# aiforvision/OCTA-autosegmentation

Measured on AMD Instinct MI355X. Metric: synthetic OCTA samples/sec (graph + 304x304 image + 1216x1216 label triples), higher is better.
Workload: dtype f64

## Files before the change

include/octa_hip.h:

```cpp
#ifndef OCTA_HIP_H
#define OCTA_HIP_H

#include <stddef.h>
#include <stdint.h>

#ifdef __cplusplus
extern "C" {
#endif

typedef struct octa_ctx octa_ctx;


int octa_abi_version(void);

const char *octa_last_error(void);

int octa_ctx_create(int device, octa_ctx **out);
void octa_ctx_destroy(octa_ctx *ctx);

size_t octa_ctx_scratch_bytes(const octa_ctx *ctx);

int octa_rasterize_2d(octa_ctx *ctx, int B, const double *d_edges, const int64_t *h_edge_off,
                      const uint8_t *d_keep, int no_pixels_x, int no_pixels_y, int mip_axis,
                      double min_radius, double max_radius, uint8_t *d_out, void *stream);
// ... 252 lines not shown

int octa_sim_edge_offsets(octa_sim *sim, int64_t *h_edge_off, int64_t *h_n_art);

int octa_sim_export_edges(octa_sim *sim, double *h_edges);

int octa_sim_export_edges_device(octa_sim *sim, double *d_edges, void *stream);

int octa_sim_trace(octa_sim *sim, int32_t *h_trace);

int octa_sim_stats(octa_sim *sim, int64_t *h_stats);

int octa_sim_kd_paths(octa_sim *sim, int64_t *h_paths);

int octa_sim_assign_paths(octa_sim *sim, int64_t *h_paths);

int octa_sim_spans(octa_sim *sim, int64_t *h_spans);

int octa_sim_timing(octa_sim *sim, double *h_out8);

int octa_sim_service_stats(octa_sim *sim, double *h_out5);

int octa_sim_geometry(int num_cus, int *h_out4);

int octa_sim_is_large(const octa_sim *sim);

int octa_sim_fields(octa_sim *sim, int sample, double *h_oxy, int64_t cap_oxy, int64_t *n_oxy, double *h_co2,
                    int64_t cap_co2, int64_t *n_co2);

int octa_sim_kat_kd_order(octa_ctx *ctx, const double *h_pts, int64_t n, const uint8_t *h_need, int32_t *h_indices);

// ... 5 lines not shown
```

octa_autosegmentation_amd/_native.py:

```python
import contextlib
import ctypes
import os
import random as _random
import threading

import numpy as np

HERE = os.path.dirname(os.path.abspath(__file__))
LIB_PATH = os.environ.get("OCTA_HIP_LIB") or os.path.join(HERE, "liboctahip.so")

_lib = None
_ctxs = {}
_lock = threading.Lock()

c_void_p, c_int, c_double, c_size_t = ctypes.c_void_p, ctypes.c_int, ctypes.c_double, ctypes.c_size_t


def _struct(name, ints, ptrs):
    fields = [("struct_size", ctypes.c_uint32)] + [(k, c_int) for k in ints.split()] + [("slope", ctypes.c_float)] + [(k, c_void_p) for k in ptrs.split()]
    return type(name, (ctypes.Structure,), {"_fields_": fields})


Conv3x3Args = _struct("Conv3x3Args", "N H W Cin Cout stride in_dilation tap_mask out_scale out_off_y out_off_x C1 CY1 nslot",
                      "d_x d_x2 d_w d_y d_y2 d_scale1 d_shift1 d_scale2 d_shift2 d_stat_partials d_stat_slots d_residual")
# ... 50 lines not shown
    "octa_sim_run_states": (c_int, [c_void_p, c_void_p, c_void_p, c_void_p, c_void_p, c_void_p, c_void_p, c_void_p]),
    "octa_sim_np_state": (c_int, [c_void_p, c_int, c_void_p]),
    "octa_thinconv_expand": (c_int, [c_void_p, c_void_p, c_void_p, c_void_p, c_void_p, c_int, c_int, c_int, c_int, c_int, c_int, c_int, ctypes.c_float, c_void_p]),
    "octa_thinconv_squeeze": (c_int, [c_void_p, c_void_p, c_void_p, c_void_p, c_void_p, c_int, c_int, c_int, c_int, c_int, c_int, c_int, c_void_p]),
    "octa_lrelu_bwd_bf16": (c_int, [c_void_p, c_void_p, c_void_p, c_void_p, ctypes.c_int64, ctypes.c_float, c_void_p]),
    "octa_thinconv_wgrad_scratch_floats": (ctypes.c_longlong, [c_int, c_int, c_int, c_int]),
    "octa_thinconv_wgrad": (c_int, [c_void_p, c_void_p, c_void_p, c_void_p, c_void_p, c_void_p, c_int, c_int, c_int, c_int, c_int, c_int, c_int, c_int, c_int, c_void_p]),
    "octa_sim_spans": (c_int, [c_void_p, c_void_p]),
    "octa_sim_edge_offsets": (c_int, [c_void_p, c_void_p, c_void_p]),
    "octa_sim_export_edges": (c_int, [c_void_p, c_void_p]),
    "octa_sim_export_edges_device": (c_int, [c_void_p, c_void_p, c_void_p]),
    "octa_sim_trace": (c_int, [c_void_p, c_void_p]),
    "octa_sim_stats": (c_int, [c_void_p, c_void_p]),
    "octa_sim_kd_paths": (c_int, [c_void_p, c_void_p]),
    "octa_sim_assign_paths": (c_int, [c_void_p, c_void_p]),
    "octa_sim_timing": (c_int, [c_void_p, c_void_p]),
    "octa_sim_service_stats": (c_int, [c_void_p, c_void_p]),
    "octa_sim_geometry": (c_int, [c_int, c_void_p]),
    "octa_sim_is_large": (c_int, [c_void_p]),
    "octa_conv2d_f32_nchw": (c_int, [c_void_p, c_void_p, c_void_p, c_void_p, c_void_p] + [c_int] * 14 + [c_void_p]),
    "octa_convtranspose2x2_f32_nchw": (c_int, [c_void_p, c_void_p, c_void_p, c_void_p, c_int, c_int, c_int, c_int, c_int, c_void_p]),
    "octa_conv2d_f32_dgrad_nchw": (c_int, [c_void_p, c_void_p, c_void_p, c_void_p] + [c_int] * 11 + [c_void_p]),
    "octa_conv2d_f32_wgrad_workspace": (c_int, [c_int] * 10 + [ctypes.POINTER(c_size_t)]),
    "octa_conv2d_f32_wgrad_nchw": (c_int, [c_void_p, c_void_p, c_void_p, c_void_p, c_void_p, c_void_p, c_size_t] + [c_int] * 10 + [c_void_p]),
    "octa_sim_fields": (c_int, [c_void_p, c_int, c_void_p, ctypes.c_int64, c_void_p, c_void_p, ctypes.c_int64, c_void_p]),
    "octa_instnorm_lrelu_nhwc_bwd": (c_int, [c_void_p, c_void_p, c_void_p, c_void_p, c_void_p, c_void_p, c_void_p, c_void_p, c_void_p, c_void_p, c_int, c_int, ctypes.c_int64, ctypes.c_float, c_void_p]),
    "octa_pack_conv_weights": (c_int, [c_void_p, c_void_p, c_int, c_void_p, c_void_p]),
    "octa_head1_nhwc_bwd": (c_int, [c_void_p, c_void_p, c_void_p, c_void_p, ctypes.c_int64, c_int, c_void_p, c_void_p, c_void_p, c_void_p]),
    "octa_instnorm_nhwc_stats": (c_int, [c_void_p, c_void_p, c_void_p, c_void_p, c_void_p, c_void_p, c_void_p, c_void_p, c_int, c_int, ctypes.c_int64, ctypes.c_float, c_void_p]),
    "octa_scale_shift_lrelu_nhwc": (c_int, [c_void_p, c_void_p, c_void_p, c_void_p, c_void_p, c_int, c_int, ctypes.c_int64, ctypes.c_float, c_void_p]),
# ... 168 lines not shown
```

octa_autosegmentation_amd/csrc/sim.hip:

```cpp

#include <chrono>
#include <vector>

#include "common.h"
#include "sim_host.h"
#include <thread>
#include <atomic>
#include <cstdlib>
#include <cstring>

using namespace OCTA_SIMK;

#if OCTA_SIM_LARGE
#define OCTA_SIM_T octa_simL_impl
#define OCTA_SIM_FN(name) octa_simL_##name
#else
#define OCTA_SIM_T octa_simS_impl
#define OCTA_SIM_FN(name) octa_simS_##name
#endif
#define octa_sim_create OCTA_SIM_FN(create)
#define octa_sim_destroy OCTA_SIM_FN(destroy)
#define octa_sim_run OCTA_SIM_FN(run)
#define octa_sim_run_states OCTA_SIM_FN(run_states)
#define octa_sim_np_state OCTA_SIM_FN(np_state)
#define octa_sim_edge_offsets OCTA_SIM_FN(edge_offsets)
#define octa_sim_export_edges OCTA_SIM_FN(export_edges)
#define octa_sim_export_edges_device OCTA_SIM_FN(export_edges_device)
#define octa_sim_trace OCTA_SIM_FN(trace)
#define octa_sim_stats OCTA_SIM_FN(stats)
#define octa_sim_kd_paths OCTA_SIM_FN(kd_paths)
#define octa_sim_assign_paths OCTA_SIM_FN(assign_paths)
#define octa_sim_fields OCTA_SIM_FN(fields)
#define octa_sim_service_stats OCTA_SIM_FN(service_stats)
#define octa_sim_geometry OCTA_SIM_FN(geometry)
#define octa_sim_spans OCTA_SIM_FN(spans)
#define octa_sim_timing OCTA_SIM_FN(timing)
#define octa_sim_kat_kd_order OCTA_SIM_FN(kat_kd_order)
struct OCTA_SIM_T;
extern "C" void octa_sim_destroy(OCTA_SIM_T *S);
extern "C" long long octa_sim_next_ticket(void);
extern "C" int *octa_sim_launch_flag(int device);

namespace {

constexpr int SIM_THREADS = SIM_THREADS_PER_WG;
constexpr int SIM_WG_PER_CU = 2;
// ... 7 lines not shown
static_assert(SIM_THREADS == 64 * KD_WAVES, "kd mailboxes are sized for KD_WAVES waves");
constexpr int REQ_CAP = 8192;

static_assert(sizeof(BifRequest) == sizeof(octa_bif_request), "request layout must match the public header");
static_assert(MAXKEPT == OCTA_BIF_MAX_ATTS, "request capacity must match the public header");

struct BatchPtrs {
    double *npos[2], *nrad[2], *nkap[2];
    int *npar[2], *nch0[2], *nch1[2];
    unsigned char *nnch[2], *nact[2];
    double *oxy, *co2, *cand, *py_u;
    unsigned *py_state;
    int *nn, *act_list;
    int *nn_prev[2];
    double *nn_d2[2];
    unsigned *sorted;
    int *gnode, *gstart, *gcount;
    Rec *rec;
    int *glist, *child_group;
    FlushRec *fl_rec;
    idx_t *kd_idx, *kd_rank;
    unsigned char *removed, *ven_near;
    unsigned long long *hashes;
    unsigned *pairs;
    unsigned long long *set_hash;
    int *set_key, *tmp_int;
    double *grid_pts;
    unsigned *cand_idx;
    double *tmp_dbl;
    SampleScalars *sc;
// ... 17 lines not shown
};

__device__ __forceinline__ SimArrays sample_arrays(const BatchPtrs &B, int s) {
    SimArrays A;
    for (int f = 0; f < 2; f++) {
        A.npos[f] = B.npos[f] + (size_t)s * NCAP * 3;
        A.nrad[f] = B.nrad[f] + (size_t)s * NCAP;
        A.nkap[f] = B.nkap[f] + (size_t)s * NCAP;
        A.npar[f] = B.npar[f] + (size_t)s * NCAP;
        A.nch0[f] = B.nch0[f] + (size_t)s * NCAP;
        A.nch1[f] = B.nch1[f] + (size_t)s * NCAP;
        A.nnch[f] = B.nnch[f] + (size_t)s * NCAP;
        A.nact[f] = B.nact[f] + (size_t)s * NCAP;
        A.nn_prev[f] = B.nn_prev[f] + (size_t)s * OCAP;
        A.nn_d2[f] = B.nn_d2[f] + (size_t)s * OCAP;
    }
    A.oxy = B.oxy + (size_t)s * OCAP * 3;
    A.co2 = B.co2 + (size_t)s * CCAP * 3;
    A.cand = B.cand + (size_t)s * NCANDCAP * 3;
    A.py_u = B.py_u + (size_t)s * PYCAP;
    A.nn = B.nn + (size_t)s * OCAP;
    A.act_list = B.act_list + (size_t)s * NCAP;
    A.sorted = B.sorted + (size_t)s * SORTCAP;
    A.gnode = B.gnode + (size_t)s * GCAP;
    A.gstart = B.gstart + (size_t)s * GCAP;
    A.gcount = B.gcount + (size_t)s * GCAP;
    A.rec = B.rec + (size_t)s * GCAP;
    A.glist = B.glist + (size_t)s * GCAP;
    A.child_group = B.child_group + (size_t)s * NCAP;
    A.fl_rec = B.fl_rec + (size_t)s * 2 * MURRAY_FLUSH_LDS;
// ... 589 lines not shown
    }
    if ((nw == 0 && cfg.forest_type == 0) || cfg.n_trees < 1 || 2 * cfg.n_trees > NCAP) { octa::set_error("octa_sim_create: bad forest config"); delete S; return -2; }
    if (std::ceil(cfg.sx * 76) > 76 || std::ceil(cfg.sy * 76) > 76) { octa::set_error("octa_sim_create: simulation space larger than the unit square"); delete S; return -2; }
    S->iters = build_iter_table(cfg, &S->C);
    BatchPtrs &P = S->P;
    memset(&P, 0, sizeof(P));
    P.C = S->C;
    const size_t nb = (size_t)B;
    int rc = 0;
    for (int f = 0; f < 2 && !rc; f++) {
        rc |= dev_alloc(S, &P.npos[f], nb * NCAP * 3); rc |= dev_alloc(S, &P.nrad[f], nb * NCAP); rc |= dev_alloc(S, &P.nkap[f], nb * NCAP);
        rc |= dev_alloc(S, &P.npar[f], nb * NCAP); rc |= dev_alloc(S, &P.nch0[f], nb * NCAP); rc |= dev_alloc(S, &P.nch1[f], nb * NCAP);
        rc |= dev_alloc(S, &P.nnch[f], nb * NCAP); rc |= dev_alloc(S, &P.nact[f], nb * NCAP);
        rc |= dev_alloc(S, &P.nn_prev[f], nb * OCAP); rc |= dev_alloc(S, &P.nn_d2[f], nb * OCAP);
    }
    rc |= dev_alloc(S, &P.oxy, nb * OCAP * 3); rc |= dev_alloc(S, &P.co2, nb * CCAP * 3);
    rc |= dev_alloc(S, &P.cand, nb * NCANDCAP * 3); rc |= dev_alloc(S, &P.py_u, nb * PYCAP); rc |= dev_alloc(S, &P.py_state, nb * 625);
    rc |= dev_alloc(S, &P.nn, nb * OCAP); rc |= dev_alloc(S, &P.act_list, nb * NCAP);
    rc |= dev_alloc(S, &P.sorted, nb * SORTCAP); rc |= dev_alloc(S, &P.gnode, nb * GCAP); rc |= dev_alloc(S, &P.gstart, nb * GCAP);
    rc |= dev_alloc(S, &P.gcount, nb * GCAP); rc |= dev_alloc(S, &P.rec, nb * GCAP);
    rc |= dev_alloc(S, &P.glist, nb * GCAP); rc |= dev_alloc(S, &P.child_group, nb * NCAP); rc |= dev_alloc(S, &P.fl_rec, nb * 2 * MURRAY_FLUSH_LDS);
    rc |= dev_alloc(S, &P.kd_idx, nb * OCAP); rc |= dev_alloc(S, &P.kd_rank, nb * OCAP);
    rc |= dev_alloc(S, &P.removed, nb * OCAP); rc |= dev_alloc(S, &P.ven_near, nb * OCAP); rc |= dev_alloc(S, &P.hashes, nb * OCAP);
    rc |= dev_alloc(S, &P.pairs, nb * PCAP); rc |= dev_alloc(S, &P.set_hash, nb * SETCAP); rc |= dev_alloc(S, &P.set_key, nb * SETCAP);
    rc |= dev_alloc(S, &P.grid_pts, nb * GRID_N * 3); rc |= dev_alloc(S, &P.cand_idx, nb * NCANDCAP);
    rc |= dev_alloc(S, &P.tmp_int, nb * (OCAP + 2 * NCANDCAP)); rc |= dev_alloc(S, &P.tmp_dbl, nb * OCAP * 3);
    rc |= dev_alloc(S, &P.sc, nb); rc |= dev_alloc(S, &P.iters, S->iters.size() + 1);
    rc |= dev_alloc(S, &P.reqs, (size_t)2 * REQ_CAP); rc |= dev_alloc(S, &P.req_count, 4); rc |= dev_alloc(S, &P.bif_results, (size_t)2 * REQ_CAP * 6);
    rc |= dev_alloc(S, &P.mt_state, nb * 625); rc |= dev_alloc(S, &P.valid_count, nb);
    if (cfg.fixed()) {
// ... 525 lines not shown
        o[0] = sc.err; o[1] = sc.py_pos; o[2] = sc.murray_steps; o[3] = sc.n_bif; o[4] = sc.respec;
        o[5] = sc.n_nodes[0]; o[6] = sc.n_nodes[1];
        memcpy(&o[7], &sc.faz_radius, 8);
        for (int k = 0; k < 16; k++) o[8 + k] = sc.prof[k];
        for (int k = 0; k < 8; k++) o[24 + k] = sc.kdprof[k];
    }
    return 0;
}

extern "C" int octa_sim_kd_paths(OCTA_SIM_T *S, int64_t *h_paths) {
    if (!S || !S->ran || !h_paths) { octa::set_error("octa_sim_kd_paths: run the simulation first"); return -2; }
    for (int s = 0; s < S->B; s++) { h_paths[2 * s] = S->h_sc[s].kd_path[0]; h_paths[2 * s + 1] = S->h_sc[s].kd_path[1]; }
    return 0;
}

extern "C" int octa_sim_assign_paths(OCTA_SIM_T *S, int64_t *h_paths) {
    if (!S || !S->ran || !h_paths) { octa::set_error("octa_sim_assign_paths: run the simulation first"); return -2; }
    for (int s = 0; s < S->B; s++) { h_paths[2 * s] = S->h_sc[s].assign_path[0]; h_paths[2 * s + 1] = S->h_sc[s].assign_path[1]; }
    return 0;
}

extern "C" int octa_sim_fields(OCTA_SIM_T *S, int sample, double *h_oxy, int64_t cap_oxy, int64_t *n_oxy, double *h_co2,
                               int64_t cap_co2, int64_t *n_co2) {
    if (!S || !S->ran || sample < 0 || sample >= S->B) { octa::set_error("octa_sim_fields: bad arguments"); return -2; }
    OCTA_HIP_CHECK(hipSetDevice(S->ctx->device));
    const SampleScalars &sc = S->h_sc[sample];
    if (n_oxy) *n_oxy = sc.n_oxy;
    if (n_co2) *n_co2 = sc.n_co2;
    if (h_oxy) {
        int64_t n = sc.n_oxy < cap_oxy ? sc.n_oxy : cap_oxy;
// ... 75 lines not shown
```

octa_autosegmentation_amd/csrc/sim_api.cpp:

```cpp
#include <cstdlib>
#include <cstring>
#include <new>

#include "common.h"

extern "C" {
struct octa_simS_impl;
struct octa_simL_impl;
#define OCTA_DECL(SFX, T)                                                                                                                       \
    int octa_sim##SFX##_create(octa_ctx *, const octa_sim_config *, int, T **);                                                                 \
    void octa_sim##SFX##_destroy(T *);                                                                                                          \
    int octa_sim##SFX##_run(T *, const uint32_t *, const uint64_t *, octa_bif_fn, void *, void *);                                              \
    int octa_sim##SFX##_run_states(T *, const double *, const double *, const uint32_t *, const uint32_t *, octa_bif_fn, void *, void *);       \
    int octa_sim##SFX##_np_state(T *, int, uint32_t *);                                                                                         \
    int octa_sim##SFX##_edge_offsets(T *, int64_t *, int64_t *);                                                                                \
    int octa_sim##SFX##_export_edges(T *, double *);                                                                                            \
    int octa_sim##SFX##_export_edges_device(T *, double *, void *);                                                                             \
    int octa_sim##SFX##_trace(T *, int32_t *);                                                                                                  \
    int octa_sim##SFX##_stats(T *, int64_t *);                                                                                                  \
    int octa_sim##SFX##_kd_paths(T *, int64_t *);                                                                                               \
    int octa_sim##SFX##_assign_paths(T *, int64_t *);                                                                                           \
    int octa_sim##SFX##_spans(T *, int64_t *);                                                                                                  \
    int octa_sim##SFX##_timing(T *, double *);                                                                                                  \
    int octa_sim##SFX##_service_stats(T *, double *);                                                                                           \
    int octa_sim##SFX##_geometry(int, int *);                                                                                                   \
    int octa_sim##SFX##_fields(T *, int, double *, int64_t, int64_t *, double *, int64_t, int64_t *);
OCTA_DECL(S, octa_simS_impl)
OCTA_DECL(L, octa_simL_impl)
#undef OCTA_DECL
int octa_simS_kat_kd_order(octa_ctx *, const double *, int64_t, const uint8_t *, int32_t *);
}

#include <atomic>
#include <mutex>
static std::atomic<long long> g_sim_launches{0};
extern "C" long long octa_sim_next_ticket(void) { return g_sim_launches.fetch_add(1, std::memory_order_acq_rel) + 1; }
// ... 57 lines not shown
extern "C" int octa_sim_run(octa_sim *sim, const uint32_t *a, const uint64_t *b, octa_bif_fn f, void *u, void *st) {
    NEED(sim, "octa_sim_run") return FWD(octa_simS_run(sim->s, a, b, f, u, st), octa_simL_run(sim->l, a, b, f, u, st));
}
extern "C" int octa_sim_run_states(octa_sim *sim, const double *fz, const double *stp, const uint32_t *a, const uint32_t *b, octa_bif_fn f, void *u, void *st) {
    NEED(sim, "octa_sim_run_states") return FWD(octa_simS_run_states(sim->s, fz, stp, a, b, f, u, st), octa_simL_run_states(sim->l, fz, stp, a, b, f, u, st));
}
extern "C" int octa_sim_np_state(octa_sim *sim, int k, uint32_t *o) { NEED(sim, "octa_sim_np_state") return FWD(octa_simS_np_state(sim->s, k, o), octa_simL_np_state(sim->l, k, o)); }
extern "C" int octa_sim_edge_offsets(octa_sim *sim, int64_t *a, int64_t *b) { NEED(sim, "octa_sim_edge_offsets") return FWD(octa_simS_edge_offsets(sim->s, a, b), octa_simL_edge_offsets(sim->l, a, b)); }
extern "C" int octa_sim_export_edges(octa_sim *sim, double *e) { NEED(sim, "octa_sim_export_edges") return FWD(octa_simS_export_edges(sim->s, e), octa_simL_export_edges(sim->l, e)); }
extern "C" int octa_sim_export_edges_device(octa_sim *sim, double *e, void *st) {
    NEED(sim, "octa_sim_export_edges_device") return FWD(octa_simS_export_edges_device(sim->s, e, st), octa_simL_export_edges_device(sim->l, e, st));
}
extern "C" int octa_sim_trace(octa_sim *sim, int32_t *t) { NEED(sim, "octa_sim_trace") return FWD(octa_simS_trace(sim->s, t), octa_simL_trace(sim->l, t)); }
extern "C" int octa_sim_stats(octa_sim *sim, int64_t *t) { NEED(sim, "octa_sim_stats") return FWD(octa_simS_stats(sim->s, t), octa_simL_stats(sim->l, t)); }
extern "C" int octa_sim_kd_paths(octa_sim *sim, int64_t *t) { NEED(sim, "octa_sim_kd_paths") return FWD(octa_simS_kd_paths(sim->s, t), octa_simL_kd_paths(sim->l, t)); }
extern "C" int octa_sim_assign_paths(octa_sim *sim, int64_t *t) { NEED(sim, "octa_sim_assign_paths") return FWD(octa_simS_assign_paths(sim->s, t), octa_simL_assign_paths(sim->l, t)); }
extern "C" int octa_sim_spans(octa_sim *sim, int64_t *t) { NEED(sim, "octa_sim_spans") return FWD(octa_simS_spans(sim->s, t), octa_simL_spans(sim->l, t)); }
extern "C" int octa_sim_timing(octa_sim *sim, double *t) { NEED(sim, "octa_sim_timing") return FWD(octa_simS_timing(sim->s, t), octa_simL_timing(sim->l, t)); }
extern "C" int octa_sim_service_stats(octa_sim *sim, double *t) { NEED(sim, "octa_sim_service_stats") return FWD(octa_simS_service_stats(sim->s, t), octa_simL_service_stats(sim->l, t)); }
extern "C" int octa_sim_fields(octa_sim *sim, int k, double *o, int64_t co, int64_t *no, double *c, int64_t cc, int64_t *nc) {
    NEED(sim, "octa_sim_fields") return FWD(octa_simS_fields(sim->s, k, o, co, no, c, cc, nc), octa_simL_fields(sim->l, k, o, co, no, c, cc, nc));
}
extern "C" int octa_sim_geometry(int num_cus, int *h_out4) { return octa_simS_geometry(num_cus, h_out4); }
extern "C" int octa_sim_kat_kd_order(octa_ctx *ctx, const double *p, int64_t n, const uint8_t *need, int32_t *o) { return octa_simS_kat_kd_order(ctx, p, n, need, o); }
extern "C" int octa_sim_is_large(const octa_sim *sim) { return sim && sim->large ? 1 : 0; }
```

octa_autosegmentation_amd/csrc/sim_core.h:

```cpp
#pragma once
#include <cmath>
#include <cstdint>
#include <cstring>
#include <algorithm>
#include "gpow.h"
#include "glibc_trig.h"

#ifndef OCTA_SIM_LARGE
#define OCTA_SIM_LARGE 0
#endif
#if OCTA_SIM_LARGE
#define OCTA_SIMK octa_simk_large
#else
#define OCTA_SIMK octa_simk
#endif
namespace OCTA_SIMK {

#if OCTA_SIM_LARGE
typedef unsigned int idx_t;
typedef unsigned long long kdw_t;
constexpr int IDX_BITS = 18;
constexpr int GROUP_BITS = 17;
constexpr int NCAP = 1 << 17;
constexpr int OCAP = 1 << 18;
constexpr int CCAP = OCAP;
constexpr int GCAP = 1 << 17;
constexpr int SORTCAP = OCAP;
constexpr int PCAP = 1 << 21;
constexpr int SETCAP = 1 << 20;
constexpr int PYCAP = 1 << 20;
// ... 91 lines not shown
    long murray_steps;
    long flush_rounds;
    long murray_deferred;
    long n_bif;
    long respec;
    long prof[16];
    long kdprof[8];
    int kd_path[2];
    int resume_it, resume_stage;
    int parked, finished;
    long t_begin, t_end;
    int fl_pending[2];
    int n_cached[2], n_nodes_cached[2];
    double delta_cached[2];
    long assign_path[2];
};

struct SimArrays {
    double *npos[2];
    double *nrad[2];
    double *nkap[2];
    int *npar[2], *nch0[2], *nch1[2];
    unsigned char *nnch[2], *nact[2];
    OCTA_HD double *npos_of(int f) const { return f ? npos[1] : npos[0]; }
    OCTA_HD double *nrad_of(int f) const { return f ? nrad[1] : nrad[0]; }
    OCTA_HD double *nkap_of(int f) const { return f ? nkap[1] : nkap[0]; }
    OCTA_HD int *npar_of(int f) const { return f ? npar[1] : npar[0]; }
    OCTA_HD int *nch0_of(int f) const { return f ? nch0[1] : nch0[0]; }
    OCTA_HD int *nch1_of(int f) const { return f ? nch1[1] : nch1[0]; }
    OCTA_HD unsigned char *nnch_of(int f) const { return f ? nnch[1] : nnch[0]; }
    OCTA_HD unsigned char *nact_of(int f) const { return f ? nact[1] : nact[0]; }
    double *oxy;
    double *co2;
    const double *cand;
    const double *py_u;
    int *nn;
    int *nn_prev[2] = {nullptr, nullptr};
    double *nn_d2[2] = {nullptr, nullptr};
    OCTA_HD int *nn_prev_of(int f) const { return f ? nn_prev[1] : nn_prev[0]; }
    OCTA_HD double *nn_d2_of(int f) const { return f ? nn_d2[1] : nn_d2[0]; }
    int *act_list;
    unsigned *sorted;
    int *gnode, *gstart, *gcount;
    Rec *rec;
    int *glist;
    int *child_group;
    FlushRec *fl_rec;
    idx_t *kd_idx, *kd_rank;
    unsigned char *removed;
    unsigned char *ven_near;
    unsigned long long *hashes;
    unsigned *pairs;
    unsigned long long *set_hash;
    int *set_key;
    double *grid_pts;
// ... 745 lines not shown
#if defined(__HIP_DEVICE_COMPILE__)
    atomicMin(p, v);
#else
    if (v < *p) *p = v;
#endif
}

constexpr int KD_TAB_OFF = OCAP * (int)sizeof(kdw_t);
constexpr int KD_BOX_BYTES = KD_RANGES * 24;
static_assert(KD_RANGES >= OCAP / 17 + 1, "ranges per level");
static_assert(KD_MAILBOX_OFF % 16 == 0 && KD_MAILBOX_OFF >= KD_TAB_OFF + KD_RANGES * KD_TAB_BYTES_PER_RANGE, "kd tables overlap the mailbox");
static_assert(KD_MAILBOX_OFF + (KD_BOX_BYTES > KD_MAILBOX_BYTES ? KD_BOX_BYTES : KD_MAILBOX_BYTES) <= SIM_USER_BYTES, "kd table layout (box table and mailbox share their area)");
OCTA_HD inline void kd_build(const Blk &b, const double *pts, int n, idx_t *out_idx, idx_t *out_rank,
                              float *xy, double zlo, double zhi, long *kdprof = nullptr, const unsigned char *need = nullptr,
                              const bool flag_in_sign = false) {
#if defined(__HIP_DEVICE_COMPILE__) && !defined(OCTA_SIM_PROF_ASSIGN) && !defined(OCTA_SIM_PROF_SAMPLE) && !defined(OCTA_SIM_PROF_SET) && !defined(OCTA_SIM_PROF_MAIL) && !defined(OCTA_SIM_PROF_SEQ) && !defined(OCTA_SIM_PROF_SEQ2)
#define KDP(slot) do { if (kdprof && b.tid == 0) { long _t = (long)wall_clock64(); kdprof[slot] += _t - _kt; _kt = _t; } } while (0)
    long _kt = (long)wall_clock64();
#else
#define KDP(slot) do { } while (0)
#endif
    kdw_t *kv = reinterpret_cast<kdw_t *>(b.user_of<1>());
    idx_t *tab = reinterpret_cast<idx_t *>(b.user_of<1>() + KD_TAB_OFF);
    idx_t *rs = tab, *re = tab + KD_RANGES;
    idx_t *rs2 = tab + 2 * KD_RANGES, *re2 = tab + 3 * KD_RANGES;
    signed char *rd = reinterpret_cast<signed char *>(tab + 4 * KD_RANGES);
    unsigned *bbf = reinterpret_cast<unsigned *>(b.user_of<1>() + KD_MAILBOX_OFF);
#if defined(__HIP_DEVICE_COMPILE__) && !OCTA_SIM_LARGE
    if ((size_t)n * (sizeof(kdw_t) + 8) + 8 <= (size_t)KD_TAB_OFF)
        xy = reinterpret_cast<float *>(b.user_of<1>() + (((size_t)n * sizeof(kdw_t) + 7) & ~(size_t)7));
#endif
// ... 252 lines not shown
constexpr int GRID_N = NCAP > OCAP ? NCAP : OCAP;
struct Grid {
    int nx, ny;
    double x0, y0, inv, cell;
    const int *cell_end;
    const idx_t *items;
    const double *spts;
    const float *sptf;
    const double *src;
};
OCTA_HD inline int grid_clampi(int v, int hi) { return v < 0 ? 0 : (v > hi ? hi : v); }
OCTA_HD inline int grid_cx(const Grid &G, double x) { return grid_clampi((int)floor((x - G.x0) * G.inv), G.nx - 1); }
OCTA_HD inline int grid_cy(const Grid &G, double y) { return grid_clampi((int)floor((y - G.y0) * G.inv), G.ny - 1); }

OCTA_HD inline Grid grid_build_once(const Blk &b, const SimArrays &A, const double *pts, const int *ids, int n, double radius, int div, bool as_float,
                                    const unsigned char *mask) {
    Grid G;
    const double span = 1.2;
    double cell = fmax(radius / div, span / GRID_MAX);
    int nc = (int)ceil(span / cell);
    if (nc < 1) nc = 1;
    if (nc > GRID_MAX) nc = GRID_MAX;
    G.nx = G.ny = nc; G.x0 = G.y0 = -0.1; G.inv = 1.0 / cell; G.cell = cell;
    const int ncell = nc * nc;
    int *hist = reinterpret_cast<int *>(b.user_of<2>());
    idx_t *items = reinterpret_cast<idx_t *>(b.user_of<2>() + (size_t)(GRID_MAX * GRID_MAX + 1) * 4);
    static_assert((size_t)(GRID_MAX * GRID_MAX + 1) * 4 + (size_t)GRID_N * sizeof(idx_t) <= (size_t)SIM_USER_BYTES, "grid table layout");
    G.cell_end = hist; G.items = items; G.spts = A.grid_pts; G.sptf = reinterpret_cast<const float *>(A.grid_pts); G.src = pts;
    if (n > GRID_N) n = GRID_N;
    b.sync();
    for (int c = b.tid; c <= ncell; c += b.nth) hist[c] = 0;
    b.sync();
    constexpr int GB = 4;
    for (int i0 = b.tid; i0 < n; i0 += GB * b.nth) {
        double px[GB], py[GB];
        bool live[GB];
#pragma unroll
        for (int k = 0; k < GB; k++) {
            const int i = i0 + k * b.nth;
            const int ic = i < n ? i : n - 1;
            const double *p = pts + 3 * (ids ? ids[ic] : ic);
            px[k] = p[0]; py[k] = p[1];
            live[k] = i < n && (!mask || mask[ic]);
// ... 20 lines not shown
        int id[GB];
        bool live[GB];
#pragma unroll
        for (int k = 0; k < GB; k++) {
            const int i = i0 + k * b.nth;
            const int ic = i < n ? i : n - 1;
            id[k] = ids ? ids[ic] : ic;
            p[k] = ld3(pts + 3 * id[k]);
            live[k] = i < n && (!mask || mask[ic]);
        }
#pragma unroll
        for (int k = 0; k < GB; k++)
            if (live[k]) {
                int pos = atomic_add_int(&hist[grid_cy(G, p[k].y) * nc + grid_cx(G, p[k].x)], 1);
                items[pos] = (idx_t)id[k];
                if (as_float) { float *f = reinterpret_cast<float *>(A.grid_pts) + 3 * pos; f[0] = (float)p[k].x; f[1] = (float)p[k].y; f[2] = (float)p[k].z; }
                else st3(A.grid_pts + 3 * pos, p[k]);
            }
    }
    b.sync();
    return G;
}
OCTA_HD inline Grid grid_build(const Blk &b, const SimArrays &A, const double *pts, const int *ids, int n, double radius, int div = 1,
                               bool as_float = false, const unsigned char *mask = nullptr) {
#if OCTA_SIM_DUP & 2
    grid_build_once(b, A, pts, ids, n, radius, div, as_float, mask);
#endif
    return grid_build_once(b, A, pts, ids, n, radius, div, as_float, mask);
}
constexpr int GRID_VB = 4;
constexpr double GRID_F_TAU = 1e-6;
struct Pt3f { float x, y, z; };
OCTA_HD inline float sqdist_f(Pt3f a, float cx, float cy, float cz) { const float dx = a.x - cx, dy = a.y - cy, dz = a.z - cz; return fmaf(dz, dz, fmaf(dy, dy, dx * dx)); }
template <bool FLT> struct GridPt;
template <> struct GridPt<false> { typedef V3 T; static OCTA_HD inline V3 load(const Grid &G, int k) { return ld3(G.spts + 3 * k); } static OCTA_HD inline V3 zero() { return v3(0, 0, 0); } };
template <> struct GridPt<true> {
    typedef Pt3f T;
    static OCTA_HD inline Pt3f load(const Grid &G, int k) { const float *f = G.sptf + 3 * k; Pt3f r = {f[0], f[1], f[2]}; return r; }
    static OCTA_HD inline Pt3f zero() { Pt3f r = {0.f, 0.f, 0.f}; return r; }
};
template <bool FLT, class F>
OCTA_HD inline void grid_visit_impl(const Grid &G, double px, double py, double radius, F &&body) {
    const int cy0 = grid_cy(G, py - radius), cy1 = grid_cy(G, py + radius);
// ... 520 lines not shown

OCTA_HD inline int add_node(const SimArrays &A, int f, V3 p, double r, int parent, double kappa, double *rad_mirror = nullptr) {
    int id = A.sc->n_nodes[f];
    if (OCTA_UNLIKELY(id >= NCAP)) { atomic_or_int(&A.sc->err, ERR_NODE_CAP); return -1; }
    A.sc->n_nodes[f] = id + 1;
    st3(A.npos_of(f) + 3 * id, p);
    A.nrad_of(f)[id] = r; A.nkap_of(f)[id] = kappa; A.npar_of(f)[id] = parent;
    if (rad_mirror) rad_mirror[id] = r;
    A.nch0_of(f)[id] = -1; A.nch1_of(f)[id] = -1; A.nnch_of(f)[id] = 0; A.nact_of(f)[id] = 1;
    if (parent >= 0) {
        int c = A.nnch_of(f)[parent];
        if (c == 0) A.nch0_of(f)[parent] = id; else if (c == 1) A.nch1_of(f)[parent] = id;
        A.nnch_of(f)[parent] = (unsigned char)(c + 1);
    }
    return id;
}

OCTA_HD inline void phase_sample(const Blk &b, const SimArrays &A, const SimConst &C, const IterParams &P, int iter) {
    SampleScalars *sc = A.sc;
    const int N = P.N;
    const double *cand = A.cand;
    (void)iter;
    const double en = fmax(P.eps_n, P.eps_k), es = P.eps_s;
    const double en2 = en * en;
    const float en_hi2f = nextafterf((float)((en + GRID_F_TAU) * (en + GRID_F_TAU)), INFINITY);
    const float es_lo2f = es > GRID_F_TAU ? nextafterf((float)((es - GRID_F_TAU) * (es - GRID_F_TAU)), -INFINITY) : 0.f;
    const float es_hi2f = nextafterf((float)((es + GRID_F_TAU) * (es + GRID_F_TAU)), INFINITY);
    const double GSd = C.gs;
    const double fcx = C.fc0 * GSd, fcy = C.fc1 * GSd, fr = sc->faz_radius * GSd * 0.5;
    int *vlist = A.tmp_int;
// ... 40 lines not shown
                        const double lim = fmin(en, oxd[j]), lo = lim - GRID_F_TAU, hi = lim + GRID_F_TAU;
                        if (lo > 0.0 && (double)d2f < lo * lo) ok = false;
                        else if (OCTA_UNLIKELY((double)d2f <= hi * hi)) {
                            const double d2 = sqdist(ld3(G.src + 3 * j), c);
                            if (d2 <= en2 && !(sqrt(d2) > oxd[j])) ok = false;
                        }
                    }
                }
            });
            okf[vi] = ok ? 1 : 0;
        }
        b.sync();
        SSP(2);
    }
    {
        Grid G = grid_build(b, A, A.oxy, nullptr, n_oxy, es, 1, true);
        SSP(3);
        for (int rep = 0; rep < ((OCTA_SIM_DUP & 8) ? 2 : 1); rep++)
        for (int vi = b.tid; vi < n_valid; vi += b.nth) {
            if (!okf[vi]) continue;
            V3 c = ld3(cand + 3 * vlist[vi]);
            bool ok = true;
            const float cxf = (float)c.x, cyf = (float)c.y, czf = (float)c.z;
            grid_visit_f(G, c.x, c.y, es, [&](int j, const Pt3f &qf) {
                if (ok) {
                    const float d2f = sqdist_f(qf, cxf, cyf, czf);
                    if (d2f < es_lo2f) ok = false;
                    else if (OCTA_UNLIKELY(d2f <= es_hi2f) && sqrt(sqdist(ld3(G.src + 3 * j), c)) <= es) ok = false;
                }
            });
            okf[vi] = ok ? 1 : 0;
// ... 1154 lines not shown
#define OCTA_SUBPROF_T0() 0L
#endif

OCTA_HD inline void phase_satisfy_art(const Blk &b, const SimArrays &A, const SimConst &C, const IterParams &P) {
    const double zext = C.sz;
    SampleScalars *sc = A.sc;
    const int nb = sc->new_begin[0], ne = sc->new_end[0];
    const int n_new = ne - nb, n_oxy = sc->n_oxy;
    if (n_new <= 0 || n_oxy <= 0) return;
    const double ek = P.eps_k, ek2 = ek * ek;
    long t0 = OCTA_SUBPROF_T0();
    for (int i = b.tid; i < n_oxy; i += b.nth) A.removed[i] = 0;
    int *ctl = b.coll() + 100;
    if (b.tid == 0) { ctl[0] = 0; ctl[1] = 0; }
    b.sync();
    {
        int *new_ids = A.tmp_int;
        for (int j = b.tid; j < n_new; j += b.nth) new_ids[j] = nb + j;
        b.sync();
        Grid G = grid_build(b, A, A.npos[0], new_ids, n_new, ek);
        for (int o = b.tid; o < n_oxy; o += b.nth) {
            const V3 p = ld3(A.oxy + 3 * o);
            grid_visit(G, p.x, p.y, ek, [&](int j, const V3 &q) {
                if (sqdist(p, q) <= ek2) {
                    int slot = atomic_add_int(&ctl[0], 1);
                    if (slot < PCAP) A.pairs[slot] = ((unsigned)(j - nb) << IDX_BITS) | (unsigned)o;
                    A.removed[o] = 1;
                }
            });
        }
        b.sync();
    }
    OCTA_SUBPROF(sc, 12, t0);
    int n_pairs = ctl[0];
    if (n_pairs > PCAP) { if (b.tid == 0) atomic_or_int(&sc->err, ERR_PAIR_CAP); n_pairs = PCAP; }
    if (n_new > (1 << (32 - IDX_BITS))) { if (b.tid == 0) atomic_or_int(&sc->err, ERR_PAIR_CAP); }
    b.sync();
    if (n_pairs == 0) return;
    {
        const int n_ven = sc->n_nodes[1];
        int *rem = A.tmp_int;
        int n_rem = 0;
        {
            const int chunk = (n_oxy + b.nth - 1) / b.nth;
            const int i0 = b.tid * chunk < n_oxy ? b.tid * chunk : n_oxy, i1 = (i0 + chunk < n_oxy) ? i0 + chunk : n_oxy;
            int local = 0;
            for (int o = i0; o < i1; o++) local += A.removed[o] ? 1 : 0;
            int ex;
            n_rem = blk_scan(b, local, &ex);
            int run = ex;
            for (int o = i0; o < i1; o++) if (A.removed[o]) rem[run++] = o;
        }
        b.sync();
        for (int k = b.tid; k < n_rem; k += b.nth) {
            const int o = rem[k];
            A.ven_near[o] = 0;
            A.hashes[o] = py_hash_tuple3(ld3(A.oxy + 3 * o));
        }
        Grid G = grid_build(b, A, A.oxy, rem, n_rem, ek);
        constexpr int VB = 4;
        for (int j0 = b.tid; j0 < n_ven; j0 += VB * b.nth) {
            V3 qv[VB];
#pragma unroll
            for (int u = 0; u < VB; u++) { const int j = j0 + u * b.nth; qv[u] = ld3(A.npos[1] + 3 * (j < n_ven ? j : n_ven - 1)); }
#pragma unroll
            for (int u = 0; u < VB; u++) {
                if (j0 + u * b.nth >= n_ven) break;
                const V3 q = qv[u];
                grid_visit(G, q.x, q.y, ek, [&](int o, const V3 &p) {
                    if (sqrt(sqdist(q, p)) <= ek) A.ven_near[o] = 1;
                });
            }
        }
        b.sync();
    }
    OCTA_SUBPROF(sc, 12, t0);
    bool set_in_lds = false, ranked = false;
#ifdef OCTA_SIM_DEBUG_SAT
    int dbg_n_ins = -1, dbg_mask = -1, dbg_base = -1;
    const int dbg_n_co2_in = sc->n_co2;
#endif
    for (int pass = 0; pass < 2; pass++) {
        ranked = pass > 0;
        if (ranked) {
            kd_build(b, A.oxy, n_oxy, A.kd_idx, A.kd_rank, reinterpret_cast<float *>(A.tmp_dbl), 0.0, zext, sc->kdprof, A.removed, true);
#if OCTA_SIM_DUP & 1
            kd_build(b, A.oxy, n_oxy, A.kd_idx, A.kd_rank, reinterpret_cast<float *>(A.tmp_dbl), 0.0, zext, nullptr, A.removed, true);
#endif
            for (int i = b.tid; i < n_pairs; i += b.nth) {
                unsigned pr = A.pairs[i];
// ... 327 lines not shown
```

Before: 1449.

## Reuse the sink grid from the sample phase in satisfied-sink removal

The sample phase now persists its float spatial grid over oxygen sinks (cell ends, items, points) in per-sample global buffers, stamped with the iteration. The satisfied-sink removal step checks the stamp. When it matches, it queries the kept grid from each new node instead of rebuilding a grid of new nodes and scanning every sink, and only the sinks added after the grid was built go through the old path. This trades extra global memory and stores per iteration for skipping a grid build and a full sink scan. Matches are screened in float with a double-precision recheck near the boundary. The large variant disables this path, and a grid-path counter export plus optional profiling hooks are added.

```diff
diff --git a/include/octa_hip.h b/include/octa_hip.h
--- a/include/octa_hip.h
+++ b/include/octa_hip.h
@@ -290,6 +290,8 @@
 
 int octa_sim_assign_paths(octa_sim *sim, int64_t *h_paths);
 
+int octa_sim_grid_paths(octa_sim *sim, int64_t *h_paths);
+
 int octa_sim_spans(octa_sim *sim, int64_t *h_spans);
 
 int octa_sim_timing(octa_sim *sim, double *h_out8);
diff --git a/octa_autosegmentation_amd/_native.py b/octa_autosegmentation_amd/_native.py
--- a/octa_autosegmentation_amd/_native.py
+++ b/octa_autosegmentation_amd/_native.py
@@ -88,6 +88,7 @@
     "octa_sim_stats": (c_int, [c_void_p, c_void_p]),
     "octa_sim_kd_paths": (c_int, [c_void_p, c_void_p]),
     "octa_sim_assign_paths": (c_int, [c_void_p, c_void_p]),
+    "octa_sim_grid_paths": (c_int, [c_void_p, c_void_p]),
     "octa_sim_timing": (c_int, [c_void_p, c_void_p]),
     "octa_sim_service_stats": (c_int, [c_void_p, c_void_p]),
     "octa_sim_geometry": (c_int, [c_int, c_void_p]),
diff --git a/octa_autosegmentation_amd/csrc/sim.hip b/octa_autosegmentation_amd/csrc/sim.hip
--- a/octa_autosegmentation_amd/csrc/sim.hip
+++ b/octa_autosegmentation_amd/csrc/sim.hip
@@ -30,6 +30,7 @@
 #define octa_sim_stats OCTA_SIM_FN(stats)
 #define octa_sim_kd_paths OCTA_SIM_FN(kd_paths)
 #define octa_sim_assign_paths OCTA_SIM_FN(assign_paths)
+#define octa_sim_grid_paths OCTA_SIM_FN(grid_paths)
 #define octa_sim_fields OCTA_SIM_FN(fields)
 #define octa_sim_service_stats OCTA_SIM_FN(service_stats)
 #define octa_sim_geometry OCTA_SIM_FN(geometry)
@@ -67,6 +68,9 @@
     int *nn, *act_list;
     int *nn_prev[2];
     double *nn_d2[2];
+    int *sg_cell;
+    idx_t *sg_items;
+    float *sg_pts;
     unsigned *sorted;
     int *gnode, *gstart, *gcount;
     Rec *rec;
@@ -114,6 +118,11 @@
         A.nact[f] = B.nact[f] + (size_t)s * NCAP;
         A.nn_prev[f] = B.nn_prev[f] + (size_t)s * OCAP;
         A.nn_d2[f] = B.nn_d2[f] + (size_t)s * OCAP;
+    }
+    if (B.sg_cell) {
+        A.sg_cell = B.sg_cell + (size_t)s * (GRID_MAX * GRID_MAX + 1);
+        A.sg_items = B.sg_items + (size_t)s * OCAP;
+        A.sg_pts = B.sg_pts + (size_t)s * OCAP * 3;
     }
     A.oxy = B.oxy + (size_t)s * OCAP * 3;
     A.co2 = B.co2 + (size_t)s * CCAP * 3;
@@ -733,6 +742,9 @@
         rc |= dev_alloc(S, &P.nnch[f], nb * NCAP); rc |= dev_alloc(S, &P.nact[f], nb * NCAP);
         rc |= dev_alloc(S, &P.nn_prev[f], nb * OCAP); rc |= dev_alloc(S, &P.nn_d2[f], nb * OCAP);
     }
+#ifndef OCTA_SIM_GRID_NOKEEP_SINK
+    rc |= dev_alloc(S, &P.sg_cell, nb * (GRID_MAX * GRID_MAX + 1)); rc |= dev_alloc(S, &P.sg_items, nb * OCAP); rc |= dev_alloc(S, &P.sg_pts, nb * OCAP * 3);
+#endif
     rc |= dev_alloc(S, &P.oxy, nb * OCAP * 3); rc |= dev_alloc(S, &P.co2, nb * CCAP * 3);
     rc |= dev_alloc(S, &P.cand, nb * NCANDCAP * 3); rc |= dev_alloc(S, &P.py_u, nb * PYCAP); rc |= dev_alloc(S, &P.py_state, nb * 625);
     rc |= dev_alloc(S, &P.nn, nb * OCAP); rc |= dev_alloc(S, &P.act_list, nb * NCAP);
@@ -1288,6 +1300,12 @@
     return 0;
 }
 
+extern "C" int octa_sim_grid_paths(OCTA_SIM_T *S, int64_t *h_paths) {
+    if (!S || !S->ran || !h_paths) { octa::set_error("octa_sim_grid_paths: run the simulation first"); return -2; }
+    for (int s = 0; s < S->B; s++) { h_paths[2 * s] = S->h_sc[s].grid_path[0]; h_paths[2 * s + 1] = S->h_sc[s].grid_path[1]; }
+    return 0;
+}
+
 extern "C" int octa_sim_assign_paths(OCTA_SIM_T *S, int64_t *h_paths) {
     if (!S || !S->ran || !h_paths) { octa::set_error("octa_sim_assign_paths: run the simulation first"); return -2; }
     for (int s = 0; s < S->B; s++) { h_paths[2 * s] = S->h_sc[s].assign_path[0]; h_paths[2 * s + 1] = S->h_sc[s].assign_path[1]; }
diff --git a/octa_autosegmentation_amd/csrc/sim_api.cpp b/octa_autosegmentation_amd/csrc/sim_api.cpp
--- a/octa_autosegmentation_amd/csrc/sim_api.cpp
+++ b/octa_autosegmentation_amd/csrc/sim_api.cpp
@@ -20,6 +20,7 @@
     int octa_sim##SFX##_stats(T *, int64_t *);                                                                                                  \
     int octa_sim##SFX##_kd_paths(T *, int64_t *);                                                                                               \
     int octa_sim##SFX##_assign_paths(T *, int64_t *);                                                                                           \
+    int octa_sim##SFX##_grid_paths(T *, int64_t *);                                                                                             \
     int octa_sim##SFX##_spans(T *, int64_t *);                                                                                                  \
     int octa_sim##SFX##_timing(T *, double *);                                                                                                  \
     int octa_sim##SFX##_service_stats(T *, double *);                                                                                           \
@@ -107,6 +108,7 @@
 extern "C" int octa_sim_trace(octa_sim *sim, int32_t *t) { NEED(sim, "octa_sim_trace") return FWD(octa_simS_trace(sim->s, t), octa_simL_trace(sim->l, t)); }
 extern "C" int octa_sim_stats(octa_sim *sim, int64_t *t) { NEED(sim, "octa_sim_stats") return FWD(octa_simS_stats(sim->s, t), octa_simL_stats(sim->l, t)); }
 extern "C" int octa_sim_kd_paths(octa_sim *sim, int64_t *t) { NEED(sim, "octa_sim_kd_paths") return FWD(octa_simS_kd_paths(sim->s, t), octa_simL_kd_paths(sim->l, t)); }
+extern "C" int octa_sim_grid_paths(octa_sim *sim, int64_t *t) { NEED(sim, "octa_sim_grid_paths") return FWD(octa_simS_grid_paths(sim->s, t), octa_simL_grid_paths(sim->l, t)); }
 extern "C" int octa_sim_assign_paths(octa_sim *sim, int64_t *t) { NEED(sim, "octa_sim_assign_paths") return FWD(octa_simS_assign_paths(sim->s, t), octa_simL_assign_paths(sim->l, t)); }
 extern "C" int octa_sim_spans(octa_sim *sim, int64_t *t) { NEED(sim, "octa_sim_spans") return FWD(octa_simS_spans(sim->s, t), octa_simL_spans(sim->l, t)); }
 extern "C" int octa_sim_timing(octa_sim *sim, double *t) { NEED(sim, "octa_sim_timing") return FWD(octa_simS_timing(sim->s, t), octa_simL_timing(sim->l, t)); }
diff --git a/octa_autosegmentation_amd/csrc/sim_core.h b/octa_autosegmentation_amd/csrc/sim_core.h
--- a/octa_autosegmentation_amd/csrc/sim_core.h
+++ b/octa_autosegmentation_amd/csrc/sim_core.h
@@ -14,6 +14,12 @@
 #else
 #define OCTA_SIMK octa_simk
 #endif
+#if defined(OCTA_SIM_GRID_NOKEEP) || OCTA_SIM_LARGE
+#ifndef OCTA_SIM_GRID_NOKEEP_SINK
+#define OCTA_SIM_GRID_NOKEEP_SINK
+#endif
+#endif
+
 namespace OCTA_SIMK {
 
 #if OCTA_SIM_LARGE
@@ -135,6 +141,9 @@
     int n_cached[2], n_nodes_cached[2];
     double delta_cached[2];
     long assign_path[2];
+    int sg_stamp, sg_n, sg_nc, sg_pad;
+    double sg_cell;
+    long grid_path[2];
 };
 
 struct SimArrays {
@@ -160,6 +169,9 @@
     double *nn_d2[2] = {nullptr, nullptr};
     OCTA_HD int *nn_prev_of(int f) const { return f ? nn_prev[1] : nn_prev[0]; }
     OCTA_HD double *nn_d2_of(int f) const { return f ? nn_d2[1] : nn_d2[0]; }
+    int *sg_cell = nullptr;
+    idx_t *sg_items = nullptr;
+    float *sg_pts = nullptr;
     int *act_list;
     unsigned *sorted;
     int *gnode, *gstart, *gcount;
@@ -935,7 +947,7 @@
 OCTA_HD inline void kd_build(const Blk &b, const double *pts, int n, idx_t *out_idx, idx_t *out_rank,
                               float *xy, double zlo, double zhi, long *kdprof = nullptr, const unsigned char *need = nullptr,
                               const bool flag_in_sign = false) {
-#if defined(__HIP_DEVICE_COMPILE__) && !defined(OCTA_SIM_PROF_ASSIGN) && !defined(OCTA_SIM_PROF_SAMPLE) && !defined(OCTA_SIM_PROF_SET) && !defined(OCTA_SIM_PROF_MAIL) && !defined(OCTA_SIM_PROF_SEQ) && !defined(OCTA_SIM_PROF_SEQ2)
+#if defined(__HIP_DEVICE_COMPILE__) && !defined(OCTA_SIM_PROF_ASSIGN) && !defined(OCTA_SIM_PROF_SAMPLE) && !defined(OCTA_SIM_PROF_SET) && !defined(OCTA_SIM_PROF_MAIL) && !defined(OCTA_SIM_PROF_SEQ) && !defined(OCTA_SIM_PROF_SEQ2) && !defined(OCTA_SIM_PROF_SAT)
 #define KDP(slot) do { if (kdprof && b.tid == 0) { long _t = (long)wall_clock64(); kdprof[slot] += _t - _kt; _kt = _t; } } while (0)
     long _kt = (long)wall_clock64();
 #else
@@ -1218,7 +1230,7 @@
 OCTA_HD inline int grid_cy(const Grid &G, double y) { return grid_clampi((int)floor((y - G.y0) * G.inv), G.ny - 1); }
 
 OCTA_HD inline Grid grid_build_once(const Blk &b, const SimArrays &A, const double *pts, const int *ids, int n, double radius, int div, bool as_float,
-                                    const unsigned char *mask) {
+                                    const unsigned char *mask, double *out_pts) {
     Grid G;
     const double span = 1.2;
     double cell = fmax(radius / div, span / GRID_MAX);
@@ -1230,7 +1242,8 @@
     int *hist = reinterpret_cast<int *>(b.user_of<2>());
     idx_t *items = reinterpret_cast<idx_t *>(b.user_of<2>() + (size_t)(GRID_MAX * GRID_MAX + 1) * 4);
     static_assert((size_t)(GRID_MAX * GRID_MAX + 1) * 4 + (size_t)GRID_N * sizeof(idx_t) <= (size_t)SIM_USER_BYTES, "grid table layout");
-    G.cell_end = hist; G.items = items; G.spts = A.grid_pts; G.sptf = reinterpret_cast<const float *>(A.grid_pts); G.src = pts;
+    double *const cpts = out_pts ? out_pts : A.grid_pts;
+    G.cell_end = hist; G.items = items; G.spts = cpts; G.sptf = reinterpret_cast<const float *>(cpts); G.src = pts;
     if (n > GRID_N) n = GRID_N;
     b.sync();
     for (int c = b.tid; c <= ncell; c += b.nth) hist[c] = 0;
@@ -1281,19 +1294,19 @@
             if (live[k]) {
                 int pos = atomic_add_int(&hist[grid_cy(G, p[k].y) * nc + grid_cx(G, p[k].x)], 1);
                 items[pos] = (idx_t)id[k];
-                if (as_float) { float *f = reinterpret_cast<float *>(A.grid_pts) + 3 * pos; f[0] = (float)p[k].x; f[1] = (float)p[k].y; f[2] = (float)p[k].z; }
-                else st3(A.grid_pts + 3 * pos, p[k]);
+                if (as_float) { float *f = reinterpret_cast<float *>(cpts) + 3 * pos; f[0] = (float)p[k].x; f[1] = (float)p[k].y; f[2] = (float)p[k].z; }
+                else st3(cpts + 3 * pos, p[k]);
             }
     }
     b.sync();
     return G;
 }
 OCTA_HD inline Grid grid_build(const Blk &b, const SimArrays &A, const double *pts, const int *ids, int n, double radius, int div = 1,
-                               bool as_float = false, const unsigned char *mask = nullptr) {
+                               bool as_float = false, const unsigned char *mask = nullptr, double *out_pts = nullptr) {
 #if OCTA_SIM_DUP & 2
-    grid_build_once(b, A, pts, ids, n, radius, div, as_float, mask);
-#endif
-    return grid_build_once(b, A, pts, ids, n, radius, div, as_float, mask);
+    grid_build_once(b, A, pts, ids, n, radius, div, as_float, mask, out_pts);
+#endif
+    return grid_build_once(b, A, pts, ids, n, radius, div, as_float, mask, out_pts);
 }
 constexpr int GRID_VB = 4;
 constexpr double GRID_F_TAU = 1e-6;
@@ -1844,6 +1857,21 @@
         A.nnch_of(f)[parent] = (unsigned char)(c + 1);
     }
     return id;
+}
+
+OCTA_HD inline Grid grid_build_sinks(const Blk &b, const SimArrays &A, int n_oxy, double es, int t) {
+#ifndef OCTA_SIM_GRID_NOKEEP_SINK
+    if (A.sg_cell != nullptr) {
+        Grid G = grid_build(b, A, A.oxy, nullptr, n_oxy, es, 1, true, nullptr, reinterpret_cast<double *>(A.sg_pts));
+        const int ncell = G.nx * G.ny;
+        for (int c = b.tid; c < ncell; c += b.nth) A.sg_cell[c] = G.cell_end[c];
+        for (int i = b.tid; i < n_oxy; i += b.nth) A.sg_items[i] = G.items[i];
+        if (b.tid == 0) { SampleScalars *sc = A.sc; sc->sg_stamp = t + 1; sc->sg_n = n_oxy; sc->sg_nc = G.nx; sc->sg_cell = G.cell; }
+        return G;
+    }
+#endif
+    (void)t;
+    return grid_build(b, A, A.oxy, nullptr, n_oxy, es, 1, true);
 }
 
 OCTA_HD inline void phase_sample(const Blk &b, const SimArrays &A, const SimConst &C, const IterParams &P, int iter) {
@@ -1914,7 +1942,7 @@
         SSP(2);
     }
     {
-        Grid G = grid_build(b, A, A.oxy, nullptr, n_oxy, es, 1, true);
+        Grid G = grid_build_sinks(b, A, n_oxy, es, P.t);
         SSP(3);
         for (int rep = 0; rep < ((OCTA_SIM_DUP & 8) ? 2 : 1); rep++)
         for (int vi = b.tid; vi < n_valid; vi += b.nth) {
@@ -3099,21 +3127,59 @@
     int *ctl = b.coll() + 100;
     if (b.tid == 0) { ctl[0] = 0; ctl[1] = 0; }
     b.sync();
+#if defined(OCTA_SIM_PROF_SAT) && defined(__HIP_DEVICE_COMPILE__)
+    long _xt = (long)wall_clock64();
+#define XSP(slot) do { if (b.tid == 0) { long _t = (long)wall_clock64(); sc->kdprof[slot] += _t - _xt; _xt = _t; } } while (0)
+#else
+#define XSP(slot) do { } while (0)
+#endif
     {
-        int *new_ids = A.tmp_int;
-        for (int j = b.tid; j < n_new; j += b.nth) new_ids[j] = nb + j;
-        b.sync();
-        Grid G = grid_build(b, A, A.npos[0], new_ids, n_new, ek);
-        for (int o = b.tid; o < n_oxy; o += b.nth) {
-            const V3 p = ld3(A.oxy + 3 * o);
-            grid_visit(G, p.x, p.y, ek, [&](int j, const V3 &q) {
-                if (sqdist(p, q) <= ek2) {
-                    int slot = atomic_add_int(&ctl[0], 1);
-                    if (slot < PCAP) A.pairs[slot] = ((unsigned)(j - nb) << IDX_BITS) | (unsigned)o;
-                    A.removed[o] = 1;
-                }
-            });
-        }
+        int o_kept = 0;
+#ifndef OCTA_SIM_GRID_NOKEEP_SINK
+        if (A.sg_cell != nullptr && sc->sg_stamp == P.t + 1 && sc->sg_n <= n_oxy) o_kept = sc->sg_n;
+        o_kept = OCTA_UNI(o_kept);
+#endif
+        if (b.tid == 0) sc->grid_path[o_kept > 0 ? 0 : 1]++;
+        if (o_kept < n_oxy) {
+            int *new_ids = A.tmp_int;
+            for (int j = b.tid; j < n_new; j += b.nth) new_ids[j] = nb + j;
+            b.sync();
+            Grid G = grid_build(b, A, A.npos[0], new_ids, n_new, ek);
+            XSP(0);
+            for (int o = o_kept + b.tid; o < n_oxy; o += b.nth) {
+                const V3 p = ld3(A.oxy + 3 * o);
+                grid_visit(G, p.x, p.y, ek, [&](int j, const V3 &q) {
+                    if (sqdist(p, q) <= ek2) {
+                        int slot = atomic_add_int(&ctl[0], 1);
+                        if (slot < PCAP) A.pairs[slot] = ((unsigned)(j - nb) << IDX_BITS) | (unsigned)o;
+                        A.removed[o] = 1;
+                    }
+                });
+            }
+            XSP(1);
+        }
+#ifndef OCTA_SIM_GRID_NOKEEP_SINK
+        if (o_kept > 0) {
+            Grid G;
+            G.nx = G.ny = OCTA_UNI(sc->sg_nc); G.x0 = G.y0 = -0.1; G.cell = sc->sg_cell; G.inv = 1.0 / G.cell;
+            G.cell_end = A.sg_cell; G.items = A.sg_items; G.spts = nullptr; G.sptf = A.sg_pts; G.src = A.oxy;
+            const float ek_hi2f = nextafterf((float)((ek + GRID_F_TAU) * (ek + GRID_F_TAU)), INFINITY);
+            const float ek_lo2f = ek > GRID_F_TAU ? nextafterf((float)((ek - GRID_F_TAU) * (ek - GRID_F_TAU)), -INFINITY) : 0.f;
+            for (int jl = b.tid; jl < n_new; jl += b.nth) {
+                const V3 q = ld3(A.npos[0] + 3 * (nb + jl));
+                const float qxf = (float)q.x, qyf = (float)q.y, qzf = (float)q.z;
+                grid_visit_f(G, q.x, q.y, ek, [&](int o, const Pt3f &pf) {
+                    const float d2f = sqdist_f(pf, qxf, qyf, qzf);
+                    if (d2f < ek_lo2f || (OCTA_UNLIKELY(d2f <= ek_hi2f) && sqdist(ld3(A.oxy + 3 * o), q) <= ek2)) {
+                        int slot = atomic_add_int(&ctl[0], 1);
+                        if (slot < PCAP) A.pairs[slot] = ((unsigned)jl << IDX_BITS) | (unsigned)o;
+                        A.removed[o] = 1;
+                    }
+                });
+            }
+            XSP(5);
+        }
+#endif
         b.sync();
     }
     OCTA_SUBPROF(sc, 12, t0);
@@ -3142,7 +3208,9 @@
             A.ven_near[o] = 0;
             A.hashes[o] = py_hash_tuple3(ld3(A.oxy + 3 * o));
         }
+        XSP(2);
         Grid G = grid_build(b, A, A.oxy, rem, n_rem, ek);
+        XSP(3);
         constexpr int VB = 4;
         for (int j0 = b.tid; j0 < n_ven; j0 += VB * b.nth) {
             V3 qv[VB];
@@ -3158,7 +3226,9 @@
             }
         }
         b.sync();
-    }
+        XSP(4);
+    }
+#undef XSP
     OCTA_SUBPROF(sc, 12, t0);
     bool set_in_lds = false, ranked = false;
 #ifdef OCTA_SIM_DEBUG_SAT
```

Result: faster. 1467 (median of 6 runs) (+1.3%).
